# Computational-Biology-TUe/conditional-ude

Measured on AMD Instinct MI355X. Metric: subject-trajectories/sec (fwd+adjoint, 3-state ODE, 30 steps), higher is better.
Workload: dtype f64

## Files before the change

conditional-ude_amd/csrc/cude_cpep.hip:

```cpp
#include "cude_device.h"
#include "cude_kernels.h"

namespace cude {

template <class Net, int NS, bool GRAD, int KEEP = 0>
__global__ __launch_bounds__(kBlock) __attribute__((amdgpu_waves_per_eu(KEEP != 0 ? 2 : 1))) void cpep_kernel(CpepArgs a) {
    constexpr int P = Net::P;
    constexpr int NC = Net::NC;
    constexpr int TABROWS = Net::HAS_TAB ? 5 * Net::NCST : 0;
    constexpr int REDROWS = TABROWS > kRedRows ? TABROWS : kRedRows;
    extern __shared__ double smem[];
    double* s_q = smem;
    double* s_red = smem + 5 * kBlock;
    double* s_tab = s_red;
    double* s_res = s_red + REDROWS * kBlock;

    const int lane = threadIdx.x;
    const int64_t gid = (int64_t)blockIdx.x * kBlock + lane;
    const bool active = gid < a.N;
    const int64_t i = active ? gid : a.N - 1;
    const int64_t N = a.N;
    const int64_t set = blockIdx.y;
    cptr_t p = as_const(a.nn + set * a.set_stride_nn);
    cptr_t phi = as_const(a.phi);
    cptr_t obs_w = as_const(a.obs_w);
    ciptr_t seg = as_const(a.seg);
    ciptr_t obs_step = as_const(a.obs_step);
    const int S = a.S, T = a.T;
    const double h = a.h;

    const double k0 = a.k0[i], k1 = a.k1[i], k2 = a.k2[i], c0 = a.c0[i];
    const double a11 = -(k0 + k2), a12 = k1, a21 = k2, a22 = -k1, f0 = k0 * c0;
    constexpr int NK = KEEP == 2 ? Net::NKEEP : 1;
    double* const act = KEEP ? a.act + (int64_t)blockIdx.x * ((int64_t)(5 * a.S + 1) * NK * kBlock) + lane : nullptr;
    double cst[NC];
    cst[0] = Net::cond_input(a.cond[set * a.set_stride_cond + i]);
    if (NC > 1) cst[1] = a.age[i];
    double c[Net::NCST];
    Net::first_layer_offset(p, cst, c);

#ifdef CUDE_WAVE_TIMING
    const long long dbg_t0 = wall_clock64();
    long long dbg_t1 = 0;
#endif
    double y1 = c0, y2 = (k2 / k1) * c0, y3 = 0.0;
    double qprev = 0.0;
    double K1a = fma(a11, y1, fma(a12, y2, f0));
    double K1b = fma(a21, y1, a22 * y2);
    int cur_seg = -1;
    double g_lo = 0.0, g_d = 0.0;
    double sse = 0.0, base = 0.0;
    double chk = fma(cst[0], 0.0, Net::param_check(p));
    if (NC > 1) chk = fma(cst[1], 0.0, chk);
    int oi = 0;
    int n = 0, s = -1;
    ciptr_t stepk = as_const(a.stepk);
    cptr_t stepd = as_const(a.stepd);
    typename Net::Exps A, E1;
    int kind = 0;
    bool run_ok = false;
#ifndef CUDE_NO_VW
    constexpr bool kVW = (GRAD && Net::HAS_VW) || KEEP != 0;
#else
    constexpr bool kVW = false;
#endif
    typename Net::VW vw;
    if constexpr (kVW) Net::load_vw(p, vw);
    const unsigned prio_par = GRAD ? (__builtin_amdgcn_s_getreg((4 << 0) | (0 << 6) | (3 << 11)) & 1u) : 0u;
    const int prio_shift = GRAD ? a.prio_shift : 0;
    if constexpr (Net::USES_TANH) tanh_tab_init(lane, !Net::LDS_BIAS);
    Net::bias_init(a.nn + set * a.set_stride_nn, lane);
#pragma unroll 1
    for (int e = -1; e < 5 * S; e++) {
        if (GRAD && prio_shift > 0) {
            if ((((unsigned)(e + 1) >> prio_shift) ^ prio_par) & 1u) __builtin_amdgcn_s_setprio(2);
            else __builtin_amdgcn_s_setprio(0);
        }
        double xv = 0.0;
        bool tab = false;
        if (e >= 0) {
            const int sg = seg[e];
            const double ph = phi[e];
            if (sg != cur_seg) {
                cur_seg = sg;
                g_lo = a.dG[(int64_t)sg * N + i];
                g_d = a.dG[(int64_t)(sg + 1) * N + i] - g_lo;
                chk = fma(g_d, 0.0, fma(g_lo, 0.0, chk));
            }
            xv = fma(ph, g_d, g_lo);
            if constexpr (Net::HAS_TAB) {
                if (s == 0) {
                    kind = stepk[3 * n];
                    if (kind == 2 && !run_ok) kind = 0;
                    if (kind == 1) {
                        const int s0 = stepk[3 * n + 2];
                        const double lo = a.dG[(int64_t)s0 * N + i];
                        const double d = a.dG[(int64_t)(s0 + 1) * N + i] - lo;
                        run_ok = !__any(!Net::tab_safe(p, c, lo, d, stepd[3 * n + 2]));
                        if (run_ok) {
                            const double cf[5] = {Tab::c(1), Tab::c(2), Tab::c(3), Tab::c(4), 1.0};
                            Net::tab_build(p, d * stepd[3 * n + 2], cf, s_tab, lane);
                            Net::tab_anchor(p, c, fma(stepd[3 * n], d, lo), A);
                        } else {
                            kind = 0;
                        }
                    } else if (kind == 2) {
#pragma unroll
                        for (int j = 0; j < Net::NCST; j++) A.v[j] *= s_tab[(4 * Net::NCST + j) * kBlock + lane];
                    }
                }
                tab = kind != 0;
                if (tab) {
#pragma unroll
                    for (int j = 0; j < Net::NCST; j++) E1.v[j] = A.v[j] * s_tab[(s * Net::NCST + j) * kBlock + lane];
                }
            }
        }
        const double x[1] = {xv};
        double v;
        if constexpr (KEEP == 2) {
            double keep[Net::NKEEP];
            v = Net::eval_vw_keep(p, vw, c, x, tab, &E1, keep);
            double* dst = act + (int64_t)(e + 1) * (Net::NKEEP * kBlock);
#pragma unroll
            for (int q = 0; q < Net::NKEEP; q++) dst[q * kBlock] = keep[q];
        } else if constexpr (KEEP == 1) {
            double sg;
            v = Net::eval_vw_sig(p, vw, c, x, tab, &E1, &sg);
            act[(int64_t)(e + 1) * kBlock] = sg;
        } else if constexpr (kVW) {
            v = Net::eval_vw(p, vw, c, x, tab, &E1);
        } else {
            v = Net::eval(p, c, x, tab, &E1);
        }
        if (e < 0) { base = v; s = 0; continue; }
        s_q[s * kBlock + lane] = v - base;
        if (++s < 5) continue;
        s = 0;
        double q[7];
        q[0] = qprev;
#pragma unroll
        for (int j = 0; j < 5; j++) q[j + 1] = s_q[j * kBlock + lane];
        q[6] = q[5];
        double K[7][2];
        K[0][0] = K1a;
        K[0][1] = K1b;
        double Y1 = y1, Y2 = y2;
#pragma unroll
        for (int st = 1; st < 7; st++) {
            double t1 = 0.0, t2 = 0.0;
#pragma unroll
            for (int j = 0; j < st; j++) {
                t1 = fma(Tab::a(st, j), K[j][0], t1);
                t2 = fma(Tab::a(st, j), K[j][1], t2);
            }
            Y1 = fma(h, t1, y1);
            Y2 = fma(h, t2, y2);
            K[st][0] = fma(a11, Y1, fma(a12, Y2, f0 + q[st]));
            K[st][1] = fma(a21, Y1, a22 * Y2);
        }
        double y3n = y3;
        if (NS == 3) {
            double t3 = 0.0;
#pragma unroll
            for (int j = 0; j < 6; j++) t3 = fma(Tab::a(6, j), q[j], t3);
            y3n = fma(h, t3, y3);
        }
        while (oi < T && obs_step[oi] == n) {
            double o1 = 0.0, o2 = 0.0, o3 = 0.0;
#pragma unroll
            for (int j = 0; j < 7; j++) {
                const double w = obs_w[oi * 7 + j];
                o1 = fma(w, K[j][0], o1);
                o2 = fma(w, K[j][1], o2);
                if (NS == 3) o3 = fma(w, q[j], o3);
            }
            o1 = fma(h, o1, y1);
            o2 = fma(h, o2, y2);
            o3 = fma(h, o3, y3);
            const double r = a.obs != nullptr ? o1 - a.obs[(int64_t)oi * N + i] : 0.0;
            sse = fma(r, r, sse);
            if (GRAD) s_res[oi * kBlock + lane] = r;
            if (a.traj != nullptr && active) {
                double* tr = a.traj + (int64_t)NS * (oi + (int64_t)T * i);
                tr[0] = o1;
                tr[1] = o2;
                if (NS == 3) tr[2] = o3;
            }
            oi++;
        }
        y1 = Y1;
        y2 = Y2;
        y3 = y3n;
        K1a = K[6][0];
        K1b = K[6][1];
        qprev = q[6];
        n++;
    }
    sse += chk;
#ifdef CUDE_WAVE_TIMING
    dbg_t1 = wall_clock64();
#endif
    const bool failed = !(fabs(sse) <= 1.79769313486231570815e308);
    if (active) {
        if (a.sse != nullptr) a.sse[set * a.set_stride_cond + i] = sse;
        if (NS == 3 && a.auc != nullptr) a.auc[i] = y3;
    }
    const double red_loss = active ? sse : 0.0;
    const double red_fail = (active && failed) ? 1.0 : 0.0;
    double* out = a.partials + ((int64_t)set * gridDim.x + blockIdx.x) * (P + 2);

    if (!GRAD) {
        const double v2[2] = {red_loss, red_fail};
        block_reduce_store<2>(v2, s_red, out + P, lane);
        return;
    } else {
        double acc[Net::NACC];
#pragma unroll
        for (int q = 0; q < Net::NACC; q++) acc[q] = 0.0;
        double dxdummy[1] = {0.0};
        double lam1 = 0.0, lam2 = 0.0;
        double kap1 = 0.0, kap2 = 0.0;
        double wtot = 0.0;
        const double gscale = 2.0 * a.inv_n;
        oi = T - 1;
        cur_seg = -1;
        n = S - 1;
        s = 4;
        double kn[NK];
        if constexpr (KEEP != 0) {
            const double* src = act + (int64_t)(5 * S) * (NK * kBlock);
#pragma unroll
            for (int q = 0; q < NK; q++) kn[q] = src[q * kBlock];
        }
#pragma unroll 1
        for (int e = 5 * S - 1; e >= -1; e--) {
            if (prio_shift > 0) {
                if ((((unsigned)(e + 1) >> prio_shift) ^ prio_par) & 1u) __builtin_amdgcn_s_setprio(2);
                else __builtin_amdgcn_s_setprio(0);
            }
                if (e >= 0 && s == 4) {
                double kb[7][2];
#pragma unroll
                for (int j = 0; j < 6; j++) { kb[j][0] = 0.0; kb[j][1] = 0.0; }
                kb[6][0] = kap1;
                kb[6][1] = kap2;
                double yb1 = 0.0, yb2 = 0.0;
                while (oi >= 0 && obs_step[oi] == n) {
                    const double g = gscale * s_res[oi * kBlock + lane];
                    yb1 += g;
                    const double hg = h * g;
#pragma unroll
                    for (int j = 0; j < 7; j++) kb[j][0] = fma(obs_w[oi * 7 + j], hg, kb[j][0]);
                    oi--;
                }
                double w[5];
                lam1 = fma(a11, kb[6][0], fma(a21, kb[6][1], lam1));
                lam2 = fma(a12, kb[6][0], fma(a22, kb[6][1], lam2));
                w[4] = kb[6][0];
                yb1 += lam1;
                yb2 += lam2;
                {
                    const double hl1 = h * lam1, hl2 = h * lam2;
#pragma unroll
                    for (int j = 0; j < 6; j++) {
                        kb[j][0] = fma(Tab::a(6, j), hl1, kb[j][0]);
                        kb[j][1] = fma(Tab::a(6, j), hl2, kb[j][1]);
                    }
                }
#pragma unroll
                for (int st = 5; st >= 1; st--) {
                    const double Yb1 = fma(a11, kb[st][0], a21 * kb[st][1]);
                    const double Yb2 = fma(a12, kb[st][0], a22 * kb[st][1]);
                    if (st == 5) w[4] += kb[5][0];
                    else w[st - 1] = kb[st][0];
                    yb1 += Yb1;
                    yb2 += Yb2;
                    const double h1 = h * Yb1, h2 = h * Yb2;
#pragma unroll
                    for (int j = 0; j < st; j++) {
                        kb[j][0] = fma(Tab::a(st, j), h1, kb[j][0]);
                        kb[j][1] = fma(Tab::a(st, j), h2, kb[j][1]);
                    }
                }
                lam1 = yb1;
                lam2 = yb2;
                kap1 = kb[0][0];
                kap2 = kb[0][1];
#pragma unroll
                for (int j = 0; j < 5; j++) s_q[j * kBlock + lane] = w[j];
                if constexpr (Net::HAS_TAB) {
                    kind = stepk[3 * n + 1];
                    if (kind == 2 && !run_ok) kind = 0;
                    if (kind == 1) {
                        const int s0 = stepk[3 * n + 2];
                        const double lo = a.dG[(int64_t)s0 * N + i];
                        const double d = a.dG[(int64_t)(s0 + 1) * N + i] - lo;
                        run_ok = !__any(!Net::tab_safe(p, c, lo, d, stepd[3 * n + 2]));
                        if (run_ok) {
                            const double cr[5] = {Tab::c(1) - 1.0, Tab::c(2) - 1.0, Tab::c(3) - 1.0, Tab::c(4) - 1.0,
                                                  -1.0};
                            Net::tab_build(p, d * stepd[3 * n + 2], cr, s_tab, lane);
                            Net::tab_anchor(p, c, fma(stepd[3 * n + 1], d, lo), A);
                        } else {
                            kind = 0;
                        }
                    } else if (kind == 2) {
#pragma unroll
                        for (int j = 0; j < Net::NCST; j++) A.v[j] *= s_tab[(4 * Net::NCST + j) * kBlock + lane];
                    }
                }
                n--;
            }
            double xv = 0.0, wv;
            bool tab = false;
            if (e >= 0) {
                const int sg = seg[e];
                const double ph = phi[e];
                if (sg != cur_seg) {
                    cur_seg = sg;
                    g_lo = a.dG[(int64_t)sg * N + i];
                    g_d = a.dG[(int64_t)(sg + 1) * N + i] - g_lo;
                }
                xv = fma(ph, g_d, g_lo);
                wv = s_q[s * kBlock + lane];
                wtot += wv;
                if constexpr (Net::HAS_TAB) {
                    tab = kind != 0;
                    if (tab) {
                        const int sr = s < 4 ? s : 0;
                        double f[Net::NCST];
#pragma unroll
                        for (int j = 0; j < Net::NCST; j++) f[j] = s_tab[(sr * Net::NCST + j) * kBlock + lane];
#pragma unroll
                        for (int j = 0; j < Net::NCST; j++) asm volatile("" : "+v"(f[j]));
#pragma unroll
                        for (int j = 0; j < Net::NCST; j++)
                            E1.v[j] = s < 4 ? A.v[j] * f[j] : A.v[j];
                    }
                }
                s = (s == 0) ? 4 : s - 1;
            } else {
                wv = -wtot;
            }
            const double x[1] = {xv};
            if constexpr (KEEP == 1) {
                const double sg = kn[0];
                if (e >= 0) kn[0] = act[(int64_t)e * kBlock];
                Net::template eval_grad_pf<false, decltype(acc), true>(p, c, x, wv, acc, dxdummy, tab, &E1, sg);
            } else if constexpr (KEEP == 2) {
                double hk[Net::DEPTH][Net::WIDTH];
#pragma unroll
                for (int l = 1; l < Net::DEPTH; l++)
#pragma unroll
                    for (int j = 0; j < Net::WIDTH; j++) hk[l][j] = kn[(l - 1) * Net::WIDTH + j];
                const double sg = kn[Net::NKEEP - 1];
                if (e >= 0) {
                    const double* src = act + (int64_t)e * (Net::NKEEP * kBlock);
#pragma unroll
                    for (int q = 0; q < Net::NKEEP; q++) kn[q] = src[q * kBlock];
                }
                Net::layer1(p, c, x, hk[0], tab, &E1);
                Net::template backward<false>(launder(p), x, hk, sg, wv, acc, dxdummy);
            } else {
                Net::template eval_grad<false>(p, c, x, wv, acc, dxdummy, tab, &E1);
            }
        }

        if (active) a.g_cond[set * a.set_stride_cond + i] = Net::grad_cond(p, acc, cst);
        block_reduce_expand<Net, NC>(acc, cst, active ? 1.0 : 0.0, red_loss, red_fail, s_red, out, lane);
#ifdef CUDE_WAVE_TIMING
        if (a.dbg != nullptr && lane == 0 && blockIdx.y == 0) {
            long long* d = a.dbg + 4 * (long long)blockIdx.x;
            d[0] = dbg_t0;
            d[1] = dbg_t1;
            d[2] = wall_clock64();
            d[3] = (long long)__builtin_amdgcn_s_getreg((4 << 0) | (0 << 6) | (31 << 11)) |
                   ((long long)__builtin_amdgcn_s_getreg((20 << 0) | (0 << 6) | (31 << 11)) << 32);
        }
#endif
    }
}

template <class Net>
constexpr bool cpep_can_keep() {
#ifdef CUDE_NO_KEEP
    return false;
#else
    return Net::HAS_VW && Net::DEPTH >= 2 && Net::HAS_TAB;
#endif
}

template <class Net, int NS, bool GRAD>
static hipError_t launch_one(const CpepArgs& a, hipStream_t s) {
    const int64_t nblocks = a.blk_count > 0 ? a.blk_count : (a.N + kBlock - 1) / kBlock;
    constexpr int TABROWS = Net::HAS_TAB ? 5 * Net::NCST : 0;
    constexpr int REDROWS = TABROWS > kRedRows ? TABROWS : kRedRows;
    const size_t lds = sizeof(double) * (size_t)(5 + REDROWS + (GRAD ? a.T : 0)) * kBlock;
    const unsigned n_sets = a.n_sets > 0 ? (unsigned)a.n_sets : 1u;
    if constexpr (GRAD && cpep_can_keep<Net>()) {
        if (a.act != nullptr && n_sets == 1) {
            if (a.keep_mode == 2)
                hipLaunchKernelGGL((cpep_kernel<Net, NS, true, 2>), dim3((unsigned)nblocks, 1), dim3(kBlock), lds, s, a);
            else
                hipLaunchKernelGGL((cpep_kernel<Net, NS, true, 1>), dim3((unsigned)nblocks, 1), dim3(kBlock), lds, s, a);
            return hipGetLastError();
        }
    }
    hipLaunchKernelGGL((cpep_kernel<Net, NS, GRAD>), dim3((unsigned)nblocks, n_sets), dim3(kBlock), lds, s, a);
    return hipGetLastError();
}

template <class Net>
static hipError_t launch_shape(int n_state, bool grad, const CpepArgs& a, hipStream_t s) {
    if (n_state == 2) return grad ? launch_one<Net, 2, true>(a, s) : launch_one<Net, 2, false>(a, s);
    if (n_state == 3) return grad ? launch_one<Net, 3, true>(a, s) : launch_one<Net, 3, false>(a, s);
    return hipErrorInvalidValue;
}

template <class Net>
static int grad_occupancy(int n_state, int T) {
    constexpr int TABROWS = Net::HAS_TAB ? 5 * Net::NCST : 0;
    constexpr int REDROWS = TABROWS > kRedRows ? TABROWS : kRedRows;
    const size_t lds = sizeof(double) * (size_t)(5 + REDROWS + T) * kBlock;
    int n = 0;
    hipError_t e = n_state == 3 ? hipOccupancyMaxActiveBlocksPerMultiprocessor(&n, cpep_kernel<Net, 3, true>, kBlock, lds)
                                : hipOccupancyMaxActiveBlocksPerMultiprocessor(&n, cpep_kernel<Net, 2, true>, kBlock, lds);
    return e == hipSuccess ? n : 0;
}
template <int NIN, int W, int D>
static hipError_t launch_general(const NetShape& net, int n_state, bool grad, const CpepArgs& a, hipStream_t s) {
#define Y(HA, OA) if (net.hact == HA && net.oact == OA) return launch_shape<CpepNetG<NIN, W, D, HA, OA>>(n_state, grad, a, s);
    CUDE_GENERAL_ACTS(Y)
#undef Y
    return hipErrorInvalidValue;
}
static bool general_shape(const NetShape& net) {
#define X(NIN, W, D) if (net.nin == NIN && net.width == W && net.depth == D) return true;
    CUDE_CPEP_GENERAL_SHAPES(X)
#undef X
    return false;
}

int cpep_grad_waves_per_cu(const NetShape& net, int n_state, int T) {
    if (net.generic()) return 1;
    if (net.symbolic()) return grad_occupancy<MmProd<false>>(n_state, T);
    if (net.general()) return 4;
#define X(NIN, W, D) if (net.nin == NIN && net.width == W && net.depth == D) return grad_occupancy<CpepNet<NIN, W, D>>(n_state, T);
    CUDE_CPEP_SHAPES(X)
#undef X
    return 0;
}

int cpep_keep_values(const NetShape& net) {
    if (net.symbolic() || net.general() || net.generic()) return 0;
#define X(NIN, W, D) if (net.nin == NIN && net.width == W && net.depth == D) return cpep_can_keep<CpepNet<NIN, W, D>>() ? CpepNet<NIN, W, D>::NKEEP : 0;
    CUDE_CPEP_SHAPES(X)
#undef X
    return 0;
}

bool cpep_shape_supported(const NetShape& net, int n_state) {
    if (net.generic()) return false;
    if (n_state != 2 && n_state != 3) return false;
    if (net.symbolic()) return true;
    if (net.general()) return general_shape(net) && general_acts_compiled(net.hact, net.oact);
#define X(NIN, W, D) if (net.nin == NIN && net.width == W && net.depth == D) return true;
    CUDE_CPEP_SHAPES(X)
#undef X
    return false;
}

hipError_t launch_cpep(const NetShape& net, int n_state, bool grad, const CpepArgs& a, hipStream_t s) {
    if (net.generic()) return launch_cpep_generic(net, n_state, grad, a, s);
    if (a.S == 0) return n_state != 2 ? hipErrorInvalidValue : launch_cpep_adaptive(net, grad, a, s);
    if (net.symbolic())
        return a.cond_raw ? launch_shape<MmProd<true>>(n_state, grad, a, s) : launch_shape<MmProd<false>>(n_state, grad, a, s);
    if (net.general()) {
#define X(NIN, W, D) if (net.nin == NIN && net.width == W && net.depth == D) return launch_general<NIN, W, D>(net, n_state, grad, a, s);
        CUDE_CPEP_GENERAL_SHAPES(X)
#undef X
        return hipErrorInvalidValue;
    }
#define X(NIN, W, D) \
    if (net.nin == NIN && net.width == W && net.depth == D) return launch_shape<CpepNet<NIN, W, D>>(n_state, grad, a, s);
    CUDE_CPEP_SHAPES(X)
#undef X
    return hipErrorInvalidValue;
}

}
```

conditional-ude_amd/csrc/cude_device.h:

```cpp
#pragma once
#include <hip/hip_runtime.h>
#include <stdint.h>

#include "cude_kernels.h"
#include "cude_math.h"

namespace cude {

__device__ __constant__ const double TS_A[7][6] = {
    {0, 0, 0, 0, 0, 0},
    {0.161, 0, 0, 0, 0, 0},
    {-0.008480655492356989, 0.335480655492357, 0, 0, 0, 0},
    {2.8971530571054935, -6.359448489975075, 4.3622954328695815, 0, 0, 0},
    {5.325864828439257, -11.748883564062828, 7.4955393428898365, -0.09249506636175525, 0, 0},
    {5.86145544294642, -12.92096931784711, 8.159367898576159, -0.071584973281401, -0.028269050394068383, 0},
    {0.09646076681806523, 0.01, 0.4798896504144996, 1.379008574103742, -3.290069515436081, 2.324710524099774}};

struct Tab {
    static constexpr double a(int i, int j) {
        constexpr double A[7][6] = {
            {0, 0, 0, 0, 0, 0},
            {0.161, 0, 0, 0, 0, 0},
            {-0.008480655492356989, 0.335480655492357, 0, 0, 0, 0},
            {2.8971530571054935, -6.359448489975075, 4.3622954328695815, 0, 0, 0},
            {5.325864828439257, -11.748883564062828, 7.4955393428898365, -0.09249506636175525, 0, 0},
            {5.86145544294642, -12.92096931784711, 8.159367898576159, -0.071584973281401, -0.028269050394068383, 0},
            {0.09646076681806523, 0.01, 0.4798896504144996, 1.379008574103742, -3.290069515436081,
             2.324710524099774}};
        return A[i][j];
    }
    static constexpr double c(int i) {
        constexpr double C[7] = {0.0, 0.161, 0.327, 0.9, 0.9800255409045097, 1.0, 1.0};
        return C[i];
    }
};

typedef const __attribute__((address_space(4))) double* cptr_t;
typedef const __attribute__((address_space(4))) int32_t* ciptr_t;
__device__ __forceinline__ cptr_t as_const(const double* p) {
    return (cptr_t)(uintptr_t)p;
}
__device__ __forceinline__ ciptr_t as_const(const int32_t* p) {
    return (ciptr_t)(uintptr_t)p;
}

__device__ __forceinline__ cptr_t launder(cptr_t p) {
    asm volatile("" : "+s"(p));
    return p;
}

#ifndef CUDE_TANH_TAB_MAXW
#define CUDE_TANH_TAB_MAXW 4
#endif
#ifdef CUDE_TANH_EXP
constexpr int kTanhTabMaxW = 0;
#else
constexpr int kTanhTabMaxW = CUDE_TANH_TAB_MAXW;
#endif
__device__ const double TANH_TAB_G[kTanhEntries] = {CUDE_TANH_TABLE_VALUES};
constexpr int kTanhRows = (kTanhEntries + 63) / 64;
__shared__ double s_tanh_tab[kTanhRows * 64];
__device__ __forceinline__ void tanh_tab_init(int lane, bool sync = true) {
#pragma unroll
    for (int r = 0; r < kTanhRows; r++) {
        const int k = lane + 64 * r;
        s_tanh_tab[k] = TANH_TAB_G[k < kTanhEntries ? k : kTanhEntries - 1];
    }
    if (sync) __syncthreads();
}
__shared__ double s_bias[64];
template <int W, int D, int L1, int LH>
__device__ __forceinline__ void bias_lds_init(const double* p, int lane) {
    static_assert((D - 1) * W <= 64, "bias row");
    if (lane < (D - 1) * W) s_bias[lane] = p[L1 + (lane / W) * LH + W * W + lane % W];
    __syncthreads();
}

template <int W, bool TT>
__device__ __forceinline__ void act_tanh_vec(const double (&z)[W], double (&t)[W]) {
    if constexpr (TT) m_tanh_vec_tab<W>(z, t, s_tanh_tab);
    else m_tanh_vec<W>(z, t);
}

template <int W, int HA, bool TT>
__device__ __forceinline__ void act_hidden_vec(const double (&z)[W], double (&h)[W]) {
    if constexpr (HA == kActHiddenTanh) {
        act_tanh_vec<W, TT>(z, h);
    } else if constexpr (HA == kActHiddenRelu) {
#pragma unroll
        for (int j = 0; j < W; j++) h[j] = fmax(z[j], 0.0);
    } else if constexpr (HA == kActHiddenSigmoid) {
        static_assert(W <= 8, "batched reciprocal");
        double e[W], d[W], pre[W];
#pragma unroll
        for (int j = 0; j < W; j++) {
            e[j] = m_exp2x(fmax(-0.5 * fabs(z[j]), -350.0));
            d[j] = 1.0 + e[j];
            pre[j] = j == 0 ? d[0] : pre[j - 1] * d[j];
        }
        double r = m_rcp(pre[W - 1]);
#pragma unroll
        for (int j = W - 1; j >= 0; j--) {
            const double inv = j > 0 ? r * pre[j - 1] : r;
            if (j > 0) r = r * d[j];
            h[j] = z[j] >= 0.0 ? inv : e[j] * inv;
        }
    } else {
#pragma unroll
        for (int j = 0; j < W; j++) h[j] = z[j];
    }
}
template <int HA>
__device__ __forceinline__ double act_hidden_deriv(double h) {
    if constexpr (HA == kActHiddenTanh) return fma(-h, h, 1.0);
    else if constexpr (HA == kActHiddenRelu) return h > 0.0 ? 1.0 : 0.0;
    else if constexpr (HA == kActHiddenSigmoid) return h * (1.0 - h);
    else return 1.0;
}
template <int OA, bool LONE>
__device__ __forceinline__ double act_out(double x, double* sig) {
    if constexpr (OA == kActOutSoftplus) {
        return m_softplus_t<LONE>(x, sig);
    } else {
        *sig = 1.0;
        return x;
    }
}

template <bool LONE>
__device__ __forceinline__ double act_softplus(double x, double* sig) { return m_softplus_t<LONE>(x, sig); }
template <bool LONE>
__device__ __forceinline__ double act_softplus_val(double x) {
    double sig;
    return m_softplus_t<LONE>(x, &sig);
}

template <int W>
struct SCol {
    double v[W];
};
template <int W>
__device__ __forceinline__ SCol<W> ld_col(cptr_t p, int off) {
    p = launder(p);
    SCol<W> c;
#pragma unroll
    for (int j = 0; j < W; j++) c.v[j] = p[off + j];
    return c;
}
template <int W>
__device__ __forceinline__ void touch(const SCol<W>& c) {
    asm volatile("" ::"s"(c.v[0]));
}
#ifndef CUDE_NO_FENCE
#define CUDE_FENCE() __builtin_amdgcn_sched_barrier(0)
#else
// ... 309 lines not shown
#else
    static constexpr bool kPinLayers = (NV > 1);
#endif
    static constexpr bool HAS_PF = (D >= 2) && !GENERAL;
    template <bool KEEP, bool SKIP_OUT = false>
    __device__ static __forceinline__ double forward_pf(cptr_t p, const double (&c)[W], const double (&x)[NV],
                                                        double (&h)[D][W], bool use_tab, const Exps* E1, SCol<W>& wo,
                                                        SCol<W * CGP>& glast) {
        double z[W];
        SCol<W> bias[D];
        SCol<W * CGP> grp[D][NG];
        double bo = 0.0;
        if constexpr (!LDS_BIAS) bias[1] = ld_col<W>(p, L1 + W * W);
        grp[1][0] = ld_col<W * CGP>(p, L1);
        CUDE_FENCE();
        if (use_tab) {
            m_tanh_from_exp<W>(E1->v, h[0]);
        } else {
#pragma unroll
            for (int i = 0; i < NV; i++) {
                const SCol<W> col = ld_col<W>(p, W * i);
#pragma unroll
                for (int j = 0; j < W; j++) z[j] = fma(col.v[j], x[i], i == 0 ? c[j] : z[j]);
            }
            act_tanh_vec<W, TT>(z, h[0]);
        }
#pragma unroll
        for (int l = 1; l < D; l++) {
            const int o = L1 + (l - 1) * LH;
#pragma unroll
            for (int j = 0; j < W; j++) z[j] = LDS_BIAS ? s_bias[(l - 1) * W + j] : seed_from_sgpr(bias[l].v[j]);
#pragma unroll
            for (int g = 0; g < NG; g++) {
                CUDE_FENCE();
                touch(grp[l][g]);
                if (g + 1 < NG) {
                    grp[l][g + 1] = ld_col<W * CGP>(p, o + W * CGP * (g + 1));
                } else if (l + 1 < D) {
                    if constexpr (!LDS_BIAS) bias[l + 1] = ld_col<W>(p, o + LH + W * W);
                    grp[l + 1][0] = ld_col<W * CGP>(p, o + LH);
                } else {
                    wo = ld_col<W>(p, OUT);
                    bo = launder(p)[OUT + W];
                }
                CUDE_FENCE();
#pragma unroll
                for (int k = 0; k < CGP; k++)
#pragma unroll
                    for (int j = 0; j < W; j++) z[j] = fma(grp[l][g].v[k * W + j], h[l - 1][g * CGP + k], z[j]);
            }
            CUDE_FENCE();
            act_tanh_vec<W, TT>(z, h[l]);
        }
        CUDE_FENCE();
        if (KEEP) glast = ld_col<W * CGP>(p, L1 + (D - 2) * LH + W * CGP * (NG - 1));
        CUDE_FENCE();
        if (SKIP_OUT) return 0.0;
        double z0 = seed_from_sgpr(bo), z1 = 0.0;
#pragma unroll
        for (int i = 0; i < W; i++) {
            if (i & 1) z1 = fma(wo.v[i], h[D - 1][i], z1);
            else z0 = fma(wo.v[i], h[D - 1][i], z0);
        }
        return z0 + z1;
    }

    template <bool WANT_DX, class A, bool SIG_IN = false, bool PIN = kPinLayers, int DX0 = 0>
    __device__ static __forceinline__ double eval_grad_pf(cptr_t p, const double (&c)[W], const double (&x)[NV],
                                                          double wgt, A& acc, double (&dx)[NV],
                                                          bool use_tab, const Exps* E1, double sig_in = 0.0) {
        p = launder(p);
        double h[D][W];
        SCol<W * CGP> grp[D][NG];
        SCol<W> wo;
        const double zo = forward_pf<true, SIG_IN>(p, c, x, h, use_tab, E1, wo, grp[D - 1][NG - 1]);
        double sig = sig_in;
        double y = 0.0;
        if (!SIG_IN) y = act_softplus<TT>(zo, &sig);
        const double dz = wgt * sig;
        acc[G_OUT + W] += dz;
        double dh[W];
#pragma unroll
        for (int i = 0; i < W; i++) {
            acc[G_OUT + i] = fma(dz, h[D - 1][i], acc[G_OUT + i]);
            dh[i] = dz * wo.v[i];
        }
#pragma unroll
        for (int l = D - 1; l >= 1; l--) {
            const int o = L1 + (l - 1) * LH;
            const int go = G_H + (l - 1) * LH;
            double d[W];
#pragma unroll
            for (int j = 0; j < W; j++) {
                d[j] = dh[j] * fma(-h[l][j], h[l][j], 1.0);
                acc[go + W * W + j] += d[j];
            }
#pragma unroll
            for (int g = NG - 1; g >= 0; g--) {
                CUDE_FENCE();
                touch(grp[l][g]);
                if (g > 0) grp[l][g - 1] = ld_col<W * CGP>(p, o + W * CGP * (g - 1));
                else if (l > 1) grp[l - 1][NG - 1] = ld_col<W * CGP>(p, o - LH + W * CGP * (NG - 1));
                CUDE_FENCE();
#pragma unroll
                for (int k = 0; k < CGP; k++) {
                    const int i = g * CGP + k;
                    double s0 = 0.0, s1 = 0.0;
#pragma unroll
                    for (int j = 0; j < W; j++) {
                        acc[go + j + W * i] = fma(d[j], h[l - 1][i], acc[go + j + W * i]);
                        if (j & 1) s1 = fma(grp[l][g].v[k * W + j], d[j], s1);
                        else s0 = fma(grp[l][g].v[k * W + j], d[j], s0);
                    }
                    dh[i] = s0 + s1;
                }
                if (PIN) {
#pragma unroll
                    for (int k = 0; k < CGP; k++)
#pragma unroll
                        for (int j = 0; j < W; j++) AccPin<A>::pin(acc, go + j + W * (g * CGP + k));
                }
            }
            if (PIN) {
#pragma unroll
                for (int j = 0; j < W; j++) AccPin<A>::pin(acc, go + W * W + j);
            }
            CUDE_FENCE();
        }
#pragma unroll
        for (int j = 0; j < W; j++) {
            const double d = dh[j] * fma(-h[0][j], h[0][j], 1.0);
            dh[j] = d;
            acc[G_C + j] += d;
#pragma unroll
            for (int i = 0; i < NV; i++) acc[G_W1V + i * W + j] = fma(d, x[i], acc[G_W1V + i * W + j]);
        }
        if (WANT_DX) {
#pragma unroll
            for (int i = DX0; i < NV; i++) {
                CUDE_FENCE();
                const SCol<W> col = ld_col<W>(p, W * i);
                double s0 = 0.0, s1 = 0.0;
#pragma unroll
                for (int j = 0; j < W; j++) {
                    if (j & 1) s1 = fma(col.v[j], dh[j], s1);
                    else s0 = fma(col.v[j], dh[j], s0);
                }
                dx[i] += s0 + s1;
            }
        }
        return y;
    }

    template <bool WANT_DX, class A, bool PIN = kPinLayers, int DX0 = 0>
    __device__ static __forceinline__ double eval_grad(cptr_t p, const double (&c)[W], const double (&x)[NV],
                                                       double wgt, A& acc, double (&dx)[NV],
                                                       bool use_tab = false, const Exps* E1 = nullptr) {
#ifndef CUDE_NO_PREFETCH
        if constexpr (HAS_PF) return eval_grad_pf<WANT_DX, A, false, PIN, DX0>(p, c, x, wgt, acc, dx, use_tab, E1);
#endif
        p = launder(p);
        double h[D][W];
        const double zo = forward(p, c, x, h, use_tab, E1);
        double sig;
        const double y = act_out<OA, TT>(zo, &sig);
        backward<WANT_DX, A, PIN, DX0>(p, x, h, sig, wgt, acc, dx);
        return y;
    }

    __device__ static __forceinline__ double eval_keep(cptr_t p, const double (&c)[W], const double (&x)[NV],
                                                       double (&h)[D][W], double* sig) {
        p = launder(p);
        return act_out<OA, TT>(forward(p, c, x, h), sig);
    }

    template <bool WANT_DX, class A, bool PIN = kPinLayers, int DX0 = 0>
    __device__ static __forceinline__ void backward(cptr_t p, const double (&x)[NV], const double (&h)[D][W], double sig,
                                                    double wgt, A& acc, double (&dx)[NV]) {
        const double dz = wgt * sig;
        acc[G_OUT + W] += dz;
        double dh[W];
        CUDE_FENCE();
        {
            const SCol<W> wo = ld_col<W>(p, OUT);
#pragma unroll
            for (int i = 0; i < W; i++) {
                acc[G_OUT + i] = fma(dz, h[D - 1][i], acc[G_OUT + i]);
                dh[i] = dz * wo.v[i];
            }
        }
#pragma unroll
        for (int l = D - 1; l >= 1; l--) {
            const int o = L1 + (l - 1) * LH;
            const int go = G_H + (l - 1) * LH;
            double d[W];
#pragma unroll
            for (int j = 0; j < W; j++) {
                d[j] = dh[j] * act_hidden_deriv<HA>(h[l][j]);
                acc[go + W * W + j] += d[j];
            }
#pragma unroll
            for (int i0 = 0; i0 < W; i0 += CG) {
                CUDE_FENCE();
                constexpr int kG = CG;
                const SCol<W * kG> col = ld_col<W * kG>(p, o + W * i0);
#pragma unroll
                for (int g = 0; g < kG; g++) {
                    const int i = i0 + g;
                    if (i < W) {
                        double s0 = 0.0, s1 = 0.0;
#pragma unroll
                        for (int j = 0; j < W; j++) {
                            acc[go + j + W * i] = fma(d[j], h[l - 1][i], acc[go + j + W * i]);
                            if (j & 1) s1 = fma(col.v[g * W + j], d[j], s1);
                            else s0 = fma(col.v[g * W + j], d[j], s0);
                        }
                        dh[i] = s0 + s1;
                        if (PIN) {
#pragma unroll
                            for (int j = 0; j < W; j++) AccPin<A>::pin(acc, go + j + W * i);
                        }
                    }
                }
            }
            if (PIN) {
#pragma unroll
                for (int j = 0; j < W; j++) AccPin<A>::pin(acc, go + W * W + j);
            }
            CUDE_FENCE();
        }
#pragma unroll
        for (int j = 0; j < W; j++) {
            const double d = dh[j] * act_hidden_deriv<HA>(h[0][j]);
            dh[j] = d;
            acc[G_C + j] += d;
#pragma unroll
            for (int i = 0; i < NV; i++) acc[G_W1V + i * W + j] = fma(d, x[i], acc[G_W1V + i * W + j]);
        }
        if (WANT_DX) {
#pragma unroll
            for (int i = DX0; i < NV; i++) {
                CUDE_FENCE();
                const SCol<W> col = ld_col<W>(p, W * i);
                double s0 = 0.0, s1 = 0.0;
#pragma unroll
                for (int j = 0; j < W; j++) {
                    if (j & 1) s1 = fma(col.v[j], dh[j], s1);
                    else s0 = fma(col.v[j], dh[j], s0);
                }
                dx[i] += s0 + s1;
            }
        }
    }

    template <class A>
    __device__ static __forceinline__ double grad_elem(int q, const A& acc,
                                                       const double (&cst)[NC > 0 ? NC : 1]) {
        if (q < W * NIN) {
            const int j = q % W, i = q / W;
            return i < NV ? acc[G_W1V + i * W + j] : acc[G_C + j] * cst[i - NV < NC ? i - NV : 0];
        }
        if (q < L1) return acc[G_C + (q - W * NIN)];
        return acc[G_H + (q - L1)];
    }
    template <class A>
    __device__ static __forceinline__ double grad_cond(cptr_t p, const A& acc,
                                                       const double (&cst)[NC > 0 ? NC : 1]) {
        double s = 0.0;
        if (NC > 0) {
#pragma unroll
            for (int j = 0; j < W; j++) s = fma(acc[G_C + j], p[j + W * NV], s);
            s *= cst[0];
        }
        return s;
    }

    __device__ static __forceinline__ void expand(cptr_t p, const double (&acc)[NACC],
                                                  const double (&cst)[NC > 0 ? NC : 1], double (&g)[P], double* dcond) {
#pragma unroll
        for (int j = 0; j < W; j++) {
#pragma unroll
            for (int i = 0; i < NV; i++) g[j + W * i] = acc[G_W1V + i * W + j];
#pragma unroll
            for (int i = 0; i < NC; i++) g[j + W * (NV + i)] = acc[G_C + j] * cst[i];
            g[W * NIN + j] = acc[G_C + j];
        }
#pragma unroll
        for (int q = 0; q < (D - 1) * LH + W + 1; q++) g[L1 + q] = acc[G_H + q];
        double s = 0.0;
        if (NC > 0) {
#pragma unroll
            for (int j = 0; j < W; j++) s = fma(acc[G_C + j], p[j + W * NV], s);
            s *= cst[0];
        }
        *dcond = s;
    }

    __device__ static __forceinline__ void cond_tangent(cptr_t p, double cst0, double (&dc)[W]) {
#pragma unroll
        for (int j = 0; j < W; j++) dc[j] = p[j + W * NV] * cst0;
    }
    template <bool HAS_DX>
    __device__ static __forceinline__ double eval_jvp(cptr_t p, const double (&c)[W], const double (&x)[NV],
                                                      const double (&dc)[W], const double (&dx)[NV], double* dy) {
        p = launder(p);
        double z[W], dz[W], h[W], dh[W];
#pragma unroll
        for (int i = 0; i < NV; i++) {
            const SCol<W> col = ld_col<W>(p, W * i);
#pragma unroll
            for (int j = 0; j < W; j++) {
                z[j] = fma(col.v[j], x[i], i == 0 ? c[j] : z[j]);
                if (HAS_DX) dz[j] = fma(col.v[j], dx[i], i == 0 ? dc[j] : dz[j]);
            }
        }
        if (!HAS_DX) {
#pragma unroll
            for (int j = 0; j < W; j++) dz[j] = dc[j];
        }
        act_hidden_vec<W, HA, TT>(z, h);
#pragma unroll
        for (int j = 0; j < W; j++) dh[j] = act_hidden_deriv<HA>(h[j]) * dz[j];
#pragma unroll
        for (int l = 1; l < D; l++) {
            const int o = L1 + (l - 1) * LH;
            CUDE_FENCE();
            if constexpr (LDS_BIAS) {
#pragma unroll
                for (int j = 0; j < W; j++) z[j] = s_bias[(l - 1) * W + j];
            } else {
                const SCol<W> b = ld_col<W>(p, o + W * W);
#pragma unroll
                for (int j = 0; j < W; j++) z[j] = seed_from_sgpr(b.v[j]);
            }
#pragma unroll
            for (int j = 0; j < W; j++) dz[j] = 0.0;
#pragma unroll
            for (int i0 = 0; i0 < W; i0 += CG) {
                CUDE_FENCE();
                constexpr int kG = CG;
                const SCol<W * kG> col = ld_col<W * kG>(p, o + W * i0);
#pragma unroll
                for (int g = 0; g < kG; g++)
#pragma unroll
                    for (int j = 0; j < W; j++)
                        if (i0 + g < W) {
                            z[j] = fma(col.v[g * W + j], h[i0 + g], z[j]);
                            dz[j] = fma(col.v[g * W + j], dh[i0 + g], dz[j]);
                        }
            }
            CUDE_FENCE();
            act_hidden_vec<W, HA, TT>(z, h);
#pragma unroll
            for (int j = 0; j < W; j++) dh[j] = act_hidden_deriv<HA>(h[j]) * dz[j];
        }
        CUDE_FENCE();
        const SCol<W> wo = ld_col<W>(p, OUT);
        double z0 = seed_from_sgpr(p[OUT + W]), z1 = 0.0, d0 = 0.0, d1 = 0.0;
#pragma unroll
        for (int i = 0; i < W; i++) {
            if (i & 1) { z1 = fma(wo.v[i], h[i], z1); d1 = fma(wo.v[i], dh[i], d1); }
            else { z0 = fma(wo.v[i], h[i], z0); d0 = fma(wo.v[i], dh[i], d0); }
        }
        double sig;
        const double y = act_out<OA, TT>(z0 + z1, &sig);
        *dy = sig * (d0 + d1);
        return y;
    }
};

#ifndef CUDE_CPEP_LDS_BIAS
#define CUDE_CPEP_LDS_BIAS 1
#endif
#ifndef CUDE_LDS_BIAS_MAXW
#define CUDE_LDS_BIAS_MAXW CUDE_TANH_TAB_MAXW
#endif
template <int NIN, int W, int D>
using CpepNet = Mlp<NIN, W, D, 1, (W <= kTanhTabMaxW && NIN == 2),
                    ((W <= kTanhTabMaxW || W <= CUDE_LDS_BIAS_MAXW) && NIN == 2 && CUDE_CPEP_LDS_BIAS != 0)>;
#ifdef CUDE_TANH_EXP
template <int W, int D>
using SuppNet = Mlp<4, W, D, 3, false>;
#else
#ifndef CUDE_SUPP_LDS_BIAS
#define CUDE_SUPP_LDS_BIAS 1
#endif
template <int W, int D>
using SuppNet = Mlp<4, W, D, 3, true, (CUDE_SUPP_LDS_BIAS != 0)>;
#endif

#define CUDE_GENERAL_ACTS(Y) Y(0, 1) Y(1, 0) Y(1, 1) Y(2, 0) Y(2, 1)
template <int NIN, int W, int D, int HA, int OA>
using CpepNetG = Mlp<NIN, W, D, 1, false, false, HA, OA>;
template <int W, int D, int HA, int OA>
using SuppNetG = Mlp<4, W, D, 3, false, false, HA, OA>;
inline bool general_acts_compiled(int hact, int oact) {
#define Y(HA, OA) if (hact == HA && oact == OA) return true;
    CUDE_GENERAL_ACTS(Y)
#undef Y
    return false;
}

#define CUDE_CPEP_SHAPES_0(X) X(2, 4, 2) X(2, 6, 2) X(3, 4, 2) X(2, 8, 2) X(2, 4, 3) X(2, 3, 2) X(2, 5, 2) X(2, 7, 2)
#define CUDE_CPEP_SHAPES_1(X) X(3, 6, 2) X(2, 4, 1) X(2, 6, 1) X(2, 6, 3) X(2, 8, 1) X(2, 8, 3) X(3, 8, 2) X(2, 3, 1)
#define CUDE_CPEP_SHAPES_2(X) X(2, 5, 1) X(2, 7, 1) X(2, 3, 3) X(2, 5, 3) X(2, 7, 3) X(3, 4, 1) X(3, 6, 1) X(3, 4, 3)
#define CUDE_CPEP_SHAPES(X) CUDE_CPEP_SHAPES_0(X) CUDE_CPEP_SHAPES_1(X) CUDE_CPEP_SHAPES_2(X)
#define CUDE_CPEP_GENERAL_SHAPES(X) X(2, 4, 2) X(2, 6, 2) X(3, 4, 2)
#define CUDE_SUPP_SHAPES(X) X(3, 5) X(3, 2) X(4, 2) X(6, 2) X(5, 2) X(3, 3) X(8, 2) X(3, 4) X(4, 3) X(4, 4) X(5, 3) X(6, 3) X(3, 1) X(4, 1) X(6, 1) X(8, 1)
#define CUDE_SUPP_GENERAL_SHAPES(X) X(3, 5) X(3, 3)

template <bool RAW>
struct MmProd {
    static constexpr bool USES_TANH = false;
    static constexpr bool LDS_BIAS = false;
    __device__ static __forceinline__ void bias_init(const double*, int) {}
    static constexpr int NC = 1, NCST = 1, P = 1;
    static constexpr int NACC = 2;
    static constexpr bool HAS_TAB = false;
    static constexpr bool HAS_VW = false;
    static constexpr bool HAS_VW_SMALL = false;
    static constexpr int DEPTH = 0, WIDTH = 1, NKEEP = 1;
    struct VW {};
    struct Exps {
        double v[1];
    };
    __device__ static __forceinline__ double cond_input(double raw) { return RAW ? raw : exp(raw); }
    __device__ static __forceinline__ void first_layer_offset(cptr_t, const double (&cst)[1], double (&c)[1]) {
        c[0] = cst[0];
    }
    __device__ static __forceinline__ double param_check(cptr_t p) { return fma(p[0], 0.0, 0.0); }
    __device__ static __forceinline__ double eval(cptr_t p, const double (&c)[1], const double (&x)[1], bool = false,
                                                  const Exps* = nullptr) {
        const double v = (p[0] * x[0]) / (x[0] + c[0]);
        return x[0] >= 0.0 ? v : 0.0;
    }
    template <bool WANT_DX, class A, bool PIN = false>
    __device__ static __forceinline__ double eval_grad(cptr_t p, const double (&c)[1], const double (&x)[1],
                                                       double wgt, A& acc, double (&dx)[1], bool = false,
                                                       const Exps* = nullptr) {
        const double r = 1.0 / (x[0] + c[0]);
        const double f = x[0] * r;
        const bool pos = x[0] >= 0.0;
        const double p0 = p[0];
        acc[0] += pos ? wgt * f : 0.0;
        acc[1] += pos ? -(wgt * p0) * f * r : 0.0;
        if (WANT_DX) dx[0] += pos ? (wgt * p0) * c[0] * r * r : 0.0;
        return pos ? p0 * f : 0.0;
    }
    __device__ static __forceinline__ void expand(cptr_t, const double (&acc)[NACC], const double (&cst)[1],
                                                  double (&g)[P], double* dcond) {
        g[0] = acc[0];
        *dcond = RAW ? acc[1] : acc[1] * cst[0];
    }
    template <class A>
    __device__ static __forceinline__ double grad_elem(int, const A& acc, const double (&)[1]) { return acc[0]; }
    template <class A>
    __device__ static __forceinline__ double grad_cond(cptr_t, const A& acc, const double (&cst)[1]) {
        return RAW ? acc[1] : acc[1] * cst[0];
    }
    __device__ static __forceinline__ void cond_tangent(cptr_t, double cst0, double (&dc)[1]) { dc[0] = RAW ? 1.0 : cst0; }
    template <bool HAS_DX>
    __device__ static __forceinline__ double eval_jvp(cptr_t p, const double (&c)[1], const double (&x)[1],
                                                      const double (&dc)[1], const double (&dx)[1], double* dy) {
        const double p0 = p[0];
        const double v = (p0 * x[0]) / (x[0] + c[0]);
        const double r = 1.0 / (x[0] + c[0]);
        double d = -(p0 * x[0]) * r * r * dc[0];
        if (HAS_DX) d = fma(p0 * c[0] * r * r, dx[0], d);
        const bool pos = x[0] >= 0.0;
        *dy = pos ? d : 0.0;
        return pos ? v : 0.0;
    }
};

template <class Net, int NHL = 0>
struct SplitAcc {
    static constexpr int HI = Net::G_OUT - NHL * Net::LH;
    static constexpr int NREG = HI - Net::G_H;
    static constexpr int NLDS = Net::NACC - NREG;
    double r[NREG > 0 ? NREG : 1];
    double* lds;
    __device__ __forceinline__ double& operator[](int q) {
        return q < Net::G_H ? lds[q * 64] : (q >= HI ? lds[(q - NREG) * 64] : r[q - Net::G_H]);
    }
    __device__ __forceinline__ const double& operator[](int q) const {
        return q < Net::G_H ? lds[q * 64] : (q >= HI ? lds[(q - NREG) * 64] : r[q - Net::G_H]);
    }
    __device__ __forceinline__ void pin(int q) {
#ifndef CUDE_NO_ACC_PIN
        if (q >= Net::G_H && q < HI) asm volatile("" : "+v"(r[q - Net::G_H]));
#endif
    }
};

constexpr int kBlockLanes = 64;
constexpr int kRedRows = 16;

template <int NV>
__device__ __forceinline__ void block_reduce_store(const double (&v)[NV], double* s_red, double* out, int lane,
                                                   double* out2 = nullptr ) {
#pragma unroll
    for (int c0 = 0; c0 < NV; c0 += kRedRows) {
        __syncthreads();
#pragma unroll
        for (int r = 0; r < kRedRows; r++)
            if (c0 + r < NV) s_red[r * kBlockLanes + lane] = v[c0 + r];
        __syncthreads();
        if (lane < kRedRows && c0 + lane < NV) {
            double acc = 0.0;
#pragma unroll 8
            for (int l = 0; l < kBlockLanes; l++) acc += s_red[lane * kBlockLanes + ((l + lane) & (kBlockLanes - 1))];
            out[c0 + lane] = acc;
            if (out2 != nullptr) out2[c0 + lane] = acc;
        }
    }
}

template <class Net, int NCST, class A>
__device__ __forceinline__ void block_reduce_expand(const A& acc, const double (&cst)[NCST], double keep,
                                                    double extra0, double extra1, double* s_red, double* out, int lane) {
    constexpr int NV = Net::P + 2;
#pragma unroll
    for (int c0 = 0; c0 < NV; c0 += kRedRows) {
        __syncthreads();
#pragma unroll
        for (int r = 0; r < kRedRows; r++) {
            const int q = c0 + r;
            if (q < Net::P) s_red[r * kBlockLanes + lane] = Net::grad_elem(q, acc, cst) * keep;
            else if (q == Net::P) s_red[r * kBlockLanes + lane] = extra0;
            else if (q == Net::P + 1) s_red[r * kBlockLanes + lane] = extra1;
        }
        __syncthreads();
        if (lane < kRedRows && c0 + lane < NV) {
            double a = 0.0;
#pragma unroll 8
            for (int l = 0; l < kBlockLanes; l++) a += s_red[lane * kBlockLanes + ((l + lane) & (kBlockLanes - 1))];
            out[c0 + lane] = a;
        }
    }
}

__device__ __forceinline__ double wave_sum(double v) {
#pragma unroll
    for (int off = 32; off >= 1; off >>= 1) v += __shfl_xor(v, off, 64);
    return v;
}

}
```

Before: 225.6 million.

## Keep hidden-layer weights register-resident across lanes via DPP broadcasts in adjoint

Result: faster. 228.1 million (median of 6 runs) (+1.1%).

```diff
diff --git a/conditional-ude_amd/csrc/cude_cpep.hip b/conditional-ude_amd/csrc/cude_cpep.hip
--- a/conditional-ude_amd/csrc/cude_cpep.hip
+++ b/conditional-ude_amd/csrc/cude_cpep.hip
@@ -4,7 +4,7 @@
 namespace cude {
 
 template <class Net, int NS, bool GRAD, int KEEP = 0>
-__global__ __launch_bounds__(kBlock) __attribute__((amdgpu_waves_per_eu(KEEP != 0 ? 2 : 1))) void cpep_kernel(CpepArgs a) {
+__global__ __launch_bounds__(kBlock) __attribute__((amdgpu_waves_per_eu((KEEP != 0 || (GRAD && Net::HAS_RW)) ? 2 : 1))) void cpep_kernel(CpepArgs a) {
     constexpr int P = Net::P;
     constexpr int NC = Net::NC;
     constexpr int TABROWS = Net::HAS_TAB ? 5 * Net::NCST : 0;
@@ -218,6 +218,13 @@
         double acc[Net::NACC];
 #pragma unroll
         for (int q = 0; q < Net::NACC; q++) acc[q] = 0.0;
+#ifndef CUDE_NO_RW
+        constexpr bool kRW = Net::HAS_RW && KEEP == 0;
+#else
+        constexpr bool kRW = false;
+#endif
+        typename Net::RW rw;
+        if constexpr (kRW) Net::load_rw(a.nn + set * a.set_stride_nn, lane, rw);
         double dxdummy[1] = {0.0};
         double lam1 = 0.0, lam2 = 0.0;
         double kap1 = 0.0, kap2 = 0.0;
@@ -314,6 +321,8 @@
             }
             double xv = 0.0, wv;
             bool tab = false;
+            typename Net::RS rs;
+            if constexpr (kRW) Net::rw_request(p, rs);
             if (e >= 0) {
                 const int sg = seg[e];
                 const double ph = phi[e];
@@ -362,13 +371,26 @@
                 }
                 Net::layer1(p, c, x, hk[0], tab, &E1);
                 Net::template backward<false>(launder(p), x, hk, sg, wv, acc, dxdummy);
+            } else if constexpr (kRW) {
+                Net::eval_grad_rw(p, rw, rs, c, x, wv, acc, tab, &E1);
             } else {
                 Net::template eval_grad<false>(p, c, x, wv, acc, dxdummy, tab, &E1);
             }
         }
 
+        if constexpr (kRW) {
+            int le = lane;
+            asm volatile("" : "+v"(le));
+            const int64_t ge = (int64_t)blockIdx.x * kBlock + le;
+            const int64_t ie = ge < a.N ? ge : a.N - 1;
+            double ce[NC];
+            ce[0] = Net::cond_input(a.cond[set * a.set_stride_cond + ie]);
+            if (active) a.g_cond[set * a.set_stride_cond + ie] = Net::grad_cond(p, acc, ce);
+            block_reduce_expand<Net, NC>(acc, ce, active ? 1.0 : 0.0, red_loss, red_fail, s_red, out, lane);
+        } else {
         if (active) a.g_cond[set * a.set_stride_cond + i] = Net::grad_cond(p, acc, cst);
         block_reduce_expand<Net, NC>(acc, cst, active ? 1.0 : 0.0, red_loss, red_fail, s_red, out, lane);
+        }
 #ifdef CUDE_WAVE_TIMING
         if (a.dbg != nullptr && lane == 0 && blockIdx.y == 0) {
             long long* d = a.dbg + 4 * (long long)blockIdx.x;
diff --git a/conditional-ude_amd/csrc/cude_device.h b/conditional-ude_amd/csrc/cude_device.h
--- a/conditional-ude_amd/csrc/cude_device.h
+++ b/conditional-ude_amd/csrc/cude_device.h
@@ -1,6 +1,8 @@
 #pragma once
 #include <hip/hip_runtime.h>
 #include <stdint.h>
+
+#include <type_traits>
 
 #include "cude_kernels.h"
 #include "cude_math.h"
@@ -616,6 +618,131 @@
         return y;
     }
 
+    static constexpr bool HAS_RW = HAS_VW && HAS_PF && HAS_TAB && !TT && D == 2 && NIN == 2 && NV == 1 && W == 6;
+    static constexpr int NRW = (W * W + W + 15) / 16;
+    struct RW {
+        double w[HAS_RW ? NRW : 1];
+    };
+    struct RS {
+        SCol<W> wo;
+        double bo;
+    };
+    __device__ static __forceinline__ void load_rw(const double* p, int lane, RW& r) {
+#pragma unroll
+        for (int k = 0; k < NRW; k++) {
+            const int q = 16 * k + (lane & 15);
+            double t = p[L1 + (q < W * W + W ? q : W * W + W - 1)];
+            asm volatile("" : "+v"(t));
+            r.w[k] = t;
+        }
+    }
+    __device__ static __forceinline__ void rw_request(cptr_t p, RS& rs) {
+        rs.wo = ld_col<W>(p, OUT);
+        rs.bo = launder(p)[OUT + W];
+    }
+    template <int Q>
+    __device__ static __forceinline__ double rw_fma(const RW& r, double b, double acc) {
+        asm("v_fmac_f64_dpp %0, %1, %2 row_newbcast:%3 row_mask:0xf bank_mask:0xf"
+            : "+v"(acc)
+            : "v"(r.w[Q / 16]), "v"(b), "n"(Q % 16));
+        return acc;
+    }
+    template <int Q>
+    __device__ static __forceinline__ double rw_get(const RW& r) {
+        double v;
+        asm("v_mov_b64_dpp %0, %1 row_newbcast:%2 row_mask:0xf bank_mask:0xf" : "=v"(v) : "v"(r.w[Q / 16]), "n"(Q % 16));
+        return v;
+    }
+    template <int I, int J, int N, class F>
+    __device__ static __forceinline__ void rw_for(F&& f) {
+        if constexpr (I < N) {
+            f(std::integral_constant<int, I>{}, std::integral_constant<int, J>{});
+            if constexpr (J + 1 < N) rw_for<I, J + 1, N>(f);
+            else rw_for<I + 1, 0, N>(f);
+        }
+    }
+    __device__ static __forceinline__ void rw_tanh(const double (&z)[W], double (&t)[W]) {
+        double d[W], pre[W];
+#pragma unroll
+        for (int j = 0; j < W; j++) {
+            double a;
+            asm("v_min_f64 %0, |%1|, %2" : "=v"(a) : "v"(z[j]), "s"(20.0));
+            d[j] = m_exp2x(a) + 1.0;
+        }
+        pre[0] = d[0];
+#pragma unroll
+        for (int j = 1; j < W; j++) pre[j] = pre[j - 1] * d[j];
+        double r = m_rcp(pre[W - 1]);
+#pragma unroll
+        for (int j = W - 1; j >= 1; j--) {
+            const double inv = r * pre[j - 1];
+            r = r * d[j];
+            t[j] = copysign(fma(-2.0, inv, 1.0), z[j]);
+        }
+        t[0] = copysign(fma(-2.0, r, 1.0), z[0]);
+    }
+    template <class A>
+    __device__ static __forceinline__ void eval_grad_rw(cptr_t p, const RW& r, const RS& rs, const double (&c)[W],
+                                                        const double (&x)[NV], double wgt, A& acc, bool use_tab,
+                                                        const Exps* E1) {
+        static_assert(HAS_RW, "resident hidden layer");
+        p = launder(p);
+        double h[2][W], z[W];
+        CUDE_FENCE();
+        if (use_tab) {
+            m_tanh_from_exp<W>(E1->v, h[0]);
+        } else {
+            const SCol<W> col = ld_col<W>(p, 0);
+#pragma unroll
+            for (int j = 0; j < W; j++) z[j] = fma(col.v[j], x[0], c[j]);
+            act_tanh_vec<W, TT>(z, h[0]);
+        }
+        rw_for<0, 0, W>([&](auto i, auto j) {
+            if constexpr (i.value == 0) z[j.value] = rw_get<W * W + j.value>(r);
+            z[j.value] = rw_fma<W * i.value + j.value>(r, h[0][i.value], z[j.value]);
+        });
+        CUDE_FENCE();
+        rw_tanh(z, h[1]);
+        CUDE_FENCE();
+        double z0 = seed_from_sgpr(rs.bo), z1 = 0.0;
+#pragma unroll
+        for (int i = 0; i < W; i++) {
+            if (i & 1) z1 = fma(rs.wo.v[i], h[1][i], z1);
+            else z0 = fma(rs.wo.v[i], h[1][i], z0);
+        }
+        double sig;
+        act_softplus<TT>(z0 + z1, &sig);
+        const double dz = wgt * sig;
+        acc[G_OUT + W] += dz;
+        double dh[W], d[W];
+#pragma unroll
+        for (int i = 0; i < W; i++) {
+            acc[G_OUT + i] = fma(dz, h[1][i], acc[G_OUT + i]);
+            dh[i] = dz * rs.wo.v[i];
+        }
+#pragma unroll
+        for (int j = 0; j < W; j++) {
+            d[j] = dh[j] * fma(-h[1][j], h[1][j], 1.0);
+            acc[G_H + W * W + j] += d[j];
+        }
+        CUDE_FENCE();
+        double s[W][2];
+        rw_for<0, 0, W>([&](auto i, auto j) {
+            constexpr int ii = W - 1 - i.value, jj = j.value;
+            acc[G_H + jj + W * ii] = fma(d[jj], h[0][ii], acc[G_H + jj + W * ii]);
+            if constexpr (jj < 2) s[ii][jj] = 0.0;
+            s[ii][jj & 1] = rw_fma<W * ii + jj>(r, d[jj], s[ii][jj & 1]);
+            if constexpr (jj == W - 1) dh[ii] = s[ii][0] + s[ii][1];
+        });
+        CUDE_FENCE();
+#pragma unroll
+        for (int j = 0; j < W; j++) {
+            const double d1 = dh[j] * fma(-h[0][j], h[0][j], 1.0);
+            acc[G_C + j] += d1;
+            acc[G_W1V + j] = fma(d1, x[0], acc[G_W1V + j]);
+        }
+    }
+
     template <bool WANT_DX, class A, bool PIN = kPinLayers, int DX0 = 0>
     __device__ static __forceinline__ double eval_grad(cptr_t p, const double (&c)[W], const double (&x)[NV],
                                                        double wgt, A& acc, double (&dx)[NV],
@@ -883,8 +1010,11 @@
     static constexpr bool HAS_TAB = false;
     static constexpr bool HAS_VW = false;
     static constexpr bool HAS_VW_SMALL = false;
+    static constexpr bool HAS_RW = false;
     static constexpr int DEPTH = 0, WIDTH = 1, NKEEP = 1;
     struct VW {};
+    struct RW {};
+    struct RS {};
     struct Exps {
         double v[1];
     };
```
